# Jackxiini/Tensorflow-distributed-learning

Hardware: AMD Instinct MI355X
Metric: images/sec (whole node) MNIST CNN global_batch=64*N (higher is better)
Workload: dtype fp32; 1 GPU; global_batch=64, parallelism=dp1, engine=fused, communicator=local, variant=reference, process_model=single, communicator_impl=LocalCommunicator, ipc_mode=dmabuf, allreduce=local, steps_per_execution=25, graph_captured=True, input_prefetch_executions=1, allreduce_in_graph=False, replicas_identical=True

## Files before the change

### csrc/kernels/mnist_cnn.hip

```cpp
#include <type_traits>

#include "common.h"
#include "mnist_cnn.h"
#include "optim.h"
#include "xgmi_device.h"

namespace tdl {

struct HeadWeights {
  float wa[10], wb[10], b4[10], b3a, b3b;
};

__device__ __forceinline__ HeadWeights load_head_weights(const MnistArgs& a, int l) {
  HeadWeights hw;
  const float* w4 = a.W + a.ow4;
#pragma unroll
  for (int c = 0; c < 10; ++c) {
    hw.wa[c] = w4[l * 10 + c];
    hw.wb[c] = w4[(l + 64) * 10 + c];
    hw.b4[c] = a.W[a.ob4 + c];
  }
  hw.b3a = a.W[a.ob3 + l];
  hw.b3b = a.W[a.ob3 + l + 64];
  return hw;
// ... 267 lines not shown
    const int mt = T >> 3, nt = T & 7, n = nt * 16 + i;
    if (mt < 100) {
      const int kf = mt * 16 + i;
      const int e4 = a.ow3 + (mt * 16 + 4 * g + (i & 3)) * 128 + nt * 16 + (i & 12);
      const f4 wold = sgd ? ld4(a.W + e4) : zero4();
      const f4 acc = quad_transpose(gemm_tn_buf(b, g, buf_rsrc(a.P2, (unsigned)(b * 1600 * 4)), 1600 * 4, kf * 4,
                                                buf_rsrc(a.dH, (unsigned)(b * 128 * 4)), 128 * 4, n * 4), i & 3);
      if (keep_g) st4(a.G + e4, acc);
      if (xdst != nullptr) st4(xdst + e4, acc);
      if (sgd) st4_sc1(buf_rsrc(a.W, (unsigned)a.nslab * 4u), e4 * 4, wold - lr * acc);
    } else {
      const float wold = sgd ? a.W[a.ob3 + n] : 0.f;
      const auto dhr = buf_rsrc(a.dH, (unsigned)(b * 128 * 4));
      const f4 acc = gemm_tn_buf<true>(b, g, dhr, 0, 0, dhr, 128 * 4, n * 4, i == 0 ? 1.f : 0.f);
      if (g == 0) {
        if (keep_g) a.G[a.ob3 + n] = acc[0];
        if (xdst != nullptr) xdst[a.ob3 + n] = acc[0];
        if (sgd) a.W[a.ob3 + n] = wold - lr * acc[0];
      }
    }
    return;
  }
  const int T3 = T - kD1TasksW3;
  if (T3 < 9) {
    const int c = min(i, 9);
    float wold[4];
#pragma unroll
    for (int r = 0; r < 4; ++r)
      wold[r] = sgd ? a.W[T3 < 8 ? a.ow4 + (T3 * 16 + 4 * g + r) * 10 + c : a.ob4 + c] : 0.f;
    const auto dlr = buf_rsrc(a.dL, (unsigned)(b * kDLStride * 4));
    const int dlc = i < 10 ? i * 4 : 0x40000000;
    const f4 acc = T3 < 8 ? gemm_tn_buf(b, g, buf_rsrc(a.H, (unsigned)(b * 128 * 4)), 128 * 4, (T3 * 16 + i) * 4, dlr,
                                        kDLStride * 4, dlc)
                          : gemm_tn_buf<true>(b, g, dlr, 0, 0, dlr, kDLStride * 4, dlc, i == 0 ? 1.f : 0.f);
    if (i < 10) {
      if (T3 < 8) {
#pragma unroll
        for (int r = 0; r < 4; ++r) {
          const int e = a.ow4 + (T3 * 16 + 4 * g + r) * 10 + i;
          if (keep_g) a.G[e] = acc[r];
          if (xdst != nullptr) xdst[e] = acc[r];
          if (sgd) a.W[e] = wold[r] - lr * acc[r];
        }
      } else if (g == 0) {
        if (keep_g) a.G[a.ob4 + i] = acc[0];
        if (xdst != nullptr) xdst[a.ob4 + i] = acc[0];
        if (sgd) a.W[a.ob4 + i] = wold[0] - lr * acc[0];
      }
    }
  }
}

__device__ __forceinline__ void dp2_task(const MnistArgs& a, int T, int lane) {
  const int i = lane & 15, g = lane >> 4;
  const int b = a.b;
  const int MT = (b + 15) >> 4;
  const int mt = T % MT, nt = T / MT;
  const int row = mt * 16 + i;
  const bool valid = row < b;
  const float* ap = a.dH + (valid ? row : 0) * 128 + 4 * g;
  const float* bp = a.W + a.ow3 + (size_t)(nt * 16 + i) * 128 + 4 * g;
  f4 av[8], bv[8];
#pragma unroll
  for (int s = 0; s < 8; ++s) {
    av[s] = ld4(ap + s * 16);
    bv[s] = ld4(bp + s * 16);
  }
  float p2v[4];
#pragma unroll
  for (int r = 0; r < 4; ++r) p2v[r] = a.P2[(size_t)min(mt * 16 + 4 * g + r, b - 1) * 1600 + nt * 16 + i];
  __builtin_amdgcn_sched_barrier(0);
  const float vm = valid ? 1.f : 0.f;
  f4 acc0 = zero4(), acc1 = zero4();
#pragma unroll
  for (int s = 0; s < 8; ++s) {
    const f4 x = av[s] * vm;
    acc0 = mfma16x16x4(x.x, bv[s].x, acc0);
    acc1 = mfma16x16x4(x.y, bv[s].y, acc1);
    acc0 = mfma16x16x4(x.z, bv[s].z, acc0);
    acc1 = mfma16x16x4(x.w, bv[s].w, acc1);
  }
  const f4 acc = acc0 + acc1;
#pragma unroll
  for (int r = 0; r < 4; ++r) {
    const int rr = mt * 16 + 4 * g + r;
    if (rr < b) a.dP2[(size_t)rr * 1600 + nt * 16 + i] = p2v[r] > 0.f ? acc[r] : 0.f;
  }
}

__global__ __launch_bounds__(256) void k_dense1_bwd(MnistArgs a, int ndp2) {
  const int T = blockIdx.x * 4 + (threadIdx.x >> 6);
  if (T < ndp2) {
    dp2_task(a, T, threadIdx.x & 63);
    return;
  }
  if (T - ndp2 < kDenseTasks) dense_w_task(a, T - ndp2, threadIdx.x & 63, false, 0.f);
}

constexpr int kP1Stride = 36;
constexpr int kDcStride = 80, kDcDim = 15, kP1StrideB = 48;
constexpr int kDgSplit = 80;
__constant__ int kWgradTiles[2][8][2] = {{{0, 6}, {6, 5}, {11, 6}, {0, 0}, {0, 0}, {0, 0}, {0, 0}, {17, 2}},
                                         {{0, 5}, {5, 5}, {10, 5}, {15, 4}, {0, 0}, {0, 0}, {0, 0}, {0, 0}}};
constexpr int kLdsDc = kDcDim * kDcDim * kDcStride;
constexpr int kLdsP1 = 169 * kP1StrideB;
constexpr int kLdsWd = 9 * 16 * 16 * 4;
constexpr int kLdsConvBwd = kLdsDc + kLdsP1 + 784 + kLdsWd + 8 * 10 * 16;

__global__ __launch_bounds__(512) void k_conv_bwd(MnistArgs a) {
  extern __shared__ __attribute__((aligned(16))) float sm[];
  float* dCs = sm;
  float* P1s = dCs + kLdsDc;
  float* Xs = P1s + kLdsP1;
  float* Wd = Xs + 784;
  float* red = Wd + kLdsWd;
  const int tid = threadIdx.x, wave = __builtin_amdgcn_readfirstlane(tid >> 6), lane = tid & 63;
  const int i = lane & 15, g = lane >> 4;
  const int bi = blockIdx.x >> 2, p = blockIdx.x & 3;
  const int h = p & 1, half = p >> 1;
  if (blockIdx.x == 0) {
    for (int r = tid; r < a.b; r += 512) a.cnt[r] = 0u;
    if (tid == 0) a.ep[0] += 1u;
  }
  stamp(a.stamps, 0);
  constexpr int kIdc = (kLdsDc / 4 + 511) / 512, kIp1 = (169 * 8 + 511) / 512, kIwd = (kLdsWd / 4 + 511) / 512;
  f4 vdc[kIdc], vp1[kIp1], vwd[kIwd], vx;
  unsigned qdc[kIdc];
  int sel[kIdc];
  const float* dpb = a.dP2 + (size_t)bi * 1600;
  const unsigned* a2b = reinterpret_cast<const unsigned*>(a.A2 + (size_t)bi * 1600);
#pragma unroll
  for (int j = 0; j < kIdc; ++j) {
    const int e4 = tid + j * 512;
    const int cell = e4 / (kDcStride / 4), c4 = e4 - cell * (kDcStride / 4);
    const int y = cell / kDcDim - 2, x = cell - (cell / kDcDim) * kDcDim - 2;
    const bool in = e4 < kLdsDc / 4 && c4 < 16 && y >= 0 && y < 10 && x >= 0 && x < 10;
    const int o = in ? ((y >> 1) * 5 + (x >> 1)) * 64 + c4 * 4 : 0;
    sel[j] = in ? (y & 1) * 2 + (x & 1) : 4;
    vdc[j] = ld4(dpb + o);
    qdc[j] = a2b[o >> 2];
  }
  const float* p1b = a.P1 + (size_t)bi * 169 * 32;
#pragma unroll
  for (int j = 0; j < kIp1; ++j) {
    const int e4 = min(tid + j * 512, 169 * 8 - 1);
    vp1[j] = ld4(p1b + (e4 >> 3) * 32 + (e4 & 7) * 4);
  }
#pragma unroll
  for (int j = 0; j < kIwd; ++j) {
    const int e4 = min(tid + j * 512, kLdsWd / 4 - 1);
    const int jj = e4 & 15, cq = (e4 >> 4) & 15, tap = e4 >> 8;
    vwd[j] = ld4(a.W + a.ow2 + (size_t)(tap * 32 + 16 * h + jj) * 64 + cq * 4);
  }
  vx = ld4(a.X + (size_t)a.idx[bi] * 784 + min(tid, 195) * 4);
  __builtin_amdgcn_sched_barrier(0);
#pragma unroll
  for (int j = 0; j < kIdc; ++j) {
    const int e4 = tid + j * 512;
    if (e4 < kLdsDc / 4) {
      const unsigned q = qdc[j];
      const unsigned s = (unsigned)sel[j];
      const f4 v = vdc[j];
      st4(dCs + e4 * 4, f4{(q & 0xffu) == s ? v.x : 0.f, ((q >> 8) & 0xffu) == s ? v.y : 0.f,
                           ((q >> 16) & 0xffu) == s ? v.z : 0.f, (q >> 24) == s ? v.w : 0.f});
    }
  }
#pragma unroll
  for (int j = 0; j < kIp1; ++j) {
    const int e4 = tid + j * 512;
    if (e4 < 169 * 8) st4(P1s + (e4 >> 3) * kP1StrideB + (e4 & 7) * 4, vp1[j]);
  }
#pragma unroll
  for (int j = 0; j < kIwd; ++j) {
    const int e4 = tid + j * 512;
    if (e4 < kLdsWd / 4) st4(Wd + e4 * 4, vwd[j]);
  }
  if (tid < 196) st4(Xs + tid * 4, vx);
  stamp(a.stamps, 1);
  __syncthreads();
  stamp(a.stamps, 2);

  {
    const int t0 = kWgradTiles[half][wave][0], ntiles = kWgradTiles[half][wave][1];
    for (int j = 0; j < ntiles; ++j) {
      const int mt = t0 + j;
      const bool bias_tile = mt == 18;
      const int k = mt * 16 + i;
      const int tap = bias_tile ? 0 : k >> 5, ci = k & 31;
      const int kh = tap / 3, kw = tap - kh * 3;
      const float* pa0 = P1s + (kh * 13 + kw + g) * kP1StrideB + ci;
      const float* paS = pa0 + (g >= 2 ? 3 * kP1StrideB : 0);
      const float* pb0 = dCs + (2 * kDcDim + 2 + g) * kDcStride + 16 * p + i;
      const float* pbS = pb0 + (g >= 2 ? 5 * kDcStride : 0);
      const float unit_a = (i == 0) ? 1.f : 0.f;
      auto kloop = [&](auto bias) {
        f4 c0 = zero4(), c1 = zero4();
#pragma unroll
        for (int s0 = 0; s0 < 25; s0 += 5) {
          float av[5], bv[5];
#pragma unroll
          for (int u = 0; u < 5; ++u) {
            const int st = s0 + u, q = (4 * st) / 10, r = (4 * st) % 10;
            const bool strad = r == 8;
            if constexpr (decltype(bias)::value) av[u] = unit_a;
            else av[u] = (strad ? paS : pa0)[(q * 13 + r) * kP1StrideB];
            bv[u] = (strad ? pbS : pb0)[(q * kDcDim + r) * kDcStride];
          }
#pragma unroll
          for (int u = 0; u < 5; ++u) {
            if ((s0 + u) & 1) c1 = mfma16x16x4(av[u], bv[u], c1);
            else c0 = mfma16x16x4(av[u], bv[u], c0);
          }
        }
        return c0 + c1;
      };
      const f4 acc = bias_tile ? kloop(std::true_type{}) : kloop(std::false_type{});
#pragma unroll
      for (int r = 0; r < 4; ++r) {
        const int row = mt * 16 + 4 * g + r;
        if (row < kMnistPart2Rows) a.part2[((size_t)bi * kMnistPart2Rows + row) * 64 + 16 * p + i] = acc[r];
      }
    }
  }

  stamp(a.stamps, 3);
  float dw[10];
#pragma unroll
  for (int j = 0; j < 10; ++j) dw[j] = 0.f;
  const int d = 7 - wave;
  const int pix0 = half ? kDgSplit : 0, pix1 = half ? 169 : kDgSplit;
  if (d < (pix1 - pix0 + 15) / 16) {
    const int P = pix0 + d * 16 + i;
    const bool valid = P < pix1;
    const int Pc = valid ? P : pix0;
    const int ih = Pc / 13, iw = Pc - ih * 13;
    const float* wb = Wd + (g * 16 + i) * 4;
    const int c = 16 * h + i;
    unsigned q1v[4];
#pragma unroll
    for (int r = 0; r < 4; ++r) {
      const int Pr = min(pix0 + d * 16 + 4 * g + r, pix1 - 1);
      q1v[r] = a.A1[((size_t)bi * 169 + Pr) * 32 + c];
    }
    const int ih_lo = (pix0 + d * 16) / 13, ih_hi = min(pix0 + d * 16 + 15, pix1 - 1) / 13;
    const int kh_lo = max(0, ih_lo - 9), kh_hi = min(2, ih_hi);
    f4 acc0 = zero4(), acc1 = zero4();
    for (int kh = kh_lo; kh <= kh_hi; ++kh) {
#pragma unroll
      for (int kw = 0; kw < 3; ++kw) {
        const int tap = kh * 3 + kw;
        const float* ap = dCs + ((ih - kh + 2) * kDcDim + (iw - kw + 2)) * kDcStride + 4 * g;
#pragma unroll
        for (int c0 = 0; c0 < 64; c0 += 16) {
          const f4 av = ld4(ap + c0);
          const f4 bv = ld4(wb + (tap * 16 + c0 / 4) * 64);
          acc0 = mfma16x16x4(av.x, bv.x, acc0);
          acc1 = mfma16x16x4(av.y, bv.y, acc1);
          acc0 = mfma16x16x4(av.z, bv.z, acc0);
          acc1 = mfma16x16x4(av.w, bv.w, acc1);
        }
      }
    }
    const f4 acc = acc0 + acc1;
    stamp(a.stamps, 6);
#pragma unroll
    for (int r = 0; r < 4; ++r) {
      const int Pr = pix0 + d * 16 + 4 * g + r;
      if (Pr < pix1) {
        const float v = P1s[Pr * kP1StrideB + c] > 0.f ? acc[r] : 0.f;
        const unsigned q1 = q1v[r];
        const int ph = Pr / 13, pw = Pr - ph * 13;
        const float* img = Xs + (2 * ph + (q1 >> 1)) * 28 + 2 * pw + (q1 & 1);
#pragma unroll
        for (int kh = 0; kh < 3; ++kh)
#pragma unroll
          for (int kw = 0; kw < 3; ++kw) dw[kh * 3 + kw] = fmaf(img[kh * 28 + kw], v, dw[kh * 3 + kw]);
        dw[9] += v;
      }
    }
  }
#pragma unroll
  for (int j = 0; j < 10; ++j) dw[j] = sum_lane_groups(dw[j]);
  if (g == 0) {
#pragma unroll
    for (int j = 0; j < 10; ++j) red[(wave * 10 + j) * 16 + i] = dw[j];
  }
  stamp(a.stamps, 4);
  __syncthreads();
  stamp(a.stamps, 5);
  if (tid < 160) {
    const int j = tid >> 4, ii = tid & 15;
    float s = 0.f;
#pragma unroll
    for (int w = 2; w < 8; ++w) s += red[(w * 10 + j) * 16 + ii];
    a.part1[((size_t)bi * 2 + half) * kMnistPart1Cols + j * 32 + 16 * h + ii] = s;
  }
}

constexpr int kLdsFwd = 784 + 320 + 169 * kP1Stride + 72 * 16 * 4 + 400 + 169 * 32 / 4 + 400 / 4 + 16 * 128 + 4 + 128 +
                        288 * 16 +
                        kHeadW;
constexpr int kDcF = 15, kDcFStride = 20;
constexpr int kLdsFwdFused = kLdsFwd + kDcF * kDcF * kDcFStride;
__constant__ int kFusedWgradTiles[8][2] = {{0, 2}, {2, 2}, {4, 3}, {7, 3}, {10, 2}, {12, 2}, {14, 2}, {16, 2}};

__device__ __forceinline__ void bwd_stamp(unsigned long long* buf, int k) {
  if (buf != nullptr && (threadIdx.x & 63) == 0)
    buf[(size_t)gridDim.x * 72 + (blockIdx.x * 8 + (threadIdx.x >> 6)) * 4 + k] = __builtin_amdgcn_s_memrealtime();
}

template <int N>
__device__ __forceinline__ void fused_wgrad_tiles(const MnistArgs& a, int bi, int cq, int t0, const float* P1s,
                                                  const float* dCs) {
  const int lane = threadIdx.x & 63, i = lane & 15, g = lane >> 4;
  const float* pa0[N];
#pragma unroll
  for (int u = 0; u < N; ++u) {
    const int k = (t0 + u) * 16 + i;
    const int tap = k >> 5, ci = k & 31;
    const int kh = tap / 3, kw = tap - kh * 3;
    pa0[u] = P1s + (kh * 13 + kw + g) * kP1Stride + ci;
  }
  const int wrapA = g >= 2 ? 3 * kP1Stride : 0, wrapB = g >= 2 ? 5 * kDcFStride : 0;
  const float* pb0 = dCs + (2 * kDcF + 2 + g) * kDcFStride + i;
  f4 acc[N];
#pragma unroll
  for (int u = 0; u < N; ++u) acc[u] = zero4();
  constexpr int kS = 3, kBlocks = (25 + kS - 1) / kS;
  float bv[2][kS], av[2][kS][N];
  auto load = [&](int buf, int blk) {
#pragma unroll
    for (int j = 0; j < kS; ++j) {
      const int st = blk * kS + j;
      if (st >= 25) break;
      const int q = (4 * st) / 10, r = (4 * st) % 10;
      const bool strad = r == 8;
      bv[buf][j] = pb0[(q * kDcF + r) * kDcFStride + (strad ? wrapB : 0)];
#pragma unroll
      for (int u = 0; u < N; ++u) av[buf][j][u] = pa0[u][(q * 13 + r) * kP1Stride + (strad ? wrapA : 0)];
    }
  };
  load(0, 0);
#pragma unroll
  for (int blk = 0; blk < kBlocks; ++blk) {
    if (blk + 1 < kBlocks) load((blk + 1) & 1, blk + 1);
    __builtin_amdgcn_sched_barrier(0);
#pragma unroll
    for (int j = 0; j < kS; ++j) {
      if (blk * kS + j >= 25) break;
#pragma unroll
      for (int u = 0; u < N; ++u) acc[u] = mfma16x16x4(av[blk & 1][j][u], bv[blk & 1][j], acc[u]);
    }
    __builtin_amdgcn_sched_barrier(0);
  }
  const auto rs = buf_rsrc(a.part2 + (size_t)bi * kP2QuadFloats, kP2QuadFloats * 4);
#pragma unroll
  for (int u = 0; u < N; ++u) st4_sc1(rs, ((((t0 + u) * 4 + g) * 64 + 16 * cq + i) * 4) * 4, acc[u]);
}

__device__ __forceinline__ void lds_dgrad_w2(const float* w2d, f4 (&bwd)[9]) {
  const int wave = __builtin_amdgcn_readfirstlane(threadIdx.x >> 6), lane = threadIdx.x & 63;
  const int i = lane & 15, g = lane >> 4, nt = wave >> 2;
#pragma unroll
  for (int tap = 0; tap < 9; ++tap) bwd[tap] = ld4(w2d + (tap * 32 + 16 * nt + i) * 16 + 4 * g);
}

__device__ __forceinline__ void fused_conv_bwd(const MnistArgs& a, int bi, int cq, const float* dp2s,
                                               const uint8_t* a2s, const float* P1s, const uint8_t* a1s,
                                               const float* xs, float* dCs, float* red, const f4 (&bwd)[9]) {
  const int tid = threadIdx.x, wave = __builtin_amdgcn_readfirstlane(tid >> 6), lane = tid & 63;
  const int i = lane & 15, g = lane >> 4;
  bwd_stamp(a.stamps, 0);

  auto wgrad = [&]() {
    const int t0 = kFusedWgradTiles[wave][0], ntiles = kFusedWgradTiles[wave][1];
    if (ntiles == 2) fused_wgrad_tiles<2>(a, bi, cq, t0, P1s, dCs);
    else fused_wgrad_tiles<3>(a, bi, cq, t0, P1s, dCs);
  };
  const bool swap = (a.variant & kMnistVariantStagger) && wave >= 4;
  if (!swap) wgrad();
  bwd_stamp(a.stamps, 1);

  float dw[10];
#pragma unroll
  for (int j = 0; j < 10; ++j) dw[j] = 0.f;
  {
    const int nt = wave >> 2, wt = wave & 3;
    const int ci = 16 * nt + i;
    constexpr int kT = 3;
    f4 acc[kT][2];
    int ih[kT], iw[kT], khlo[kT], khhi[kT];
#pragma unroll
    for (int u = 0; u < kT; ++u) {
      const int t = wt + 4 * u;
      const int Pc = min(t * 16 + i, 168);
      ih[u] = Pc / 13;
      iw[u] = Pc - ih[u] * 13;
      const int ih_lo = min(t * 16, 168) / 13, ih_hi = min(t * 16 + 15, 168) / 13;
      khlo[u] = t < 11 ? max(0, ih_lo - 9) : 3;
      khhi[u] = min(2, ih_hi);
      acc[u][0] = zero4();
      acc[u][1] = zero4();
    }
    float p1v[kT][4];
    unsigned q1v[kT][4];
#pragma unroll
    for (int u = 0; u < kT; ++u)
#pragma unroll
      for (int r = 0; r < 4; ++r) {
        const int Pr = min((wt + 4 * u) * 16 + 4 * g + r, 168);
        p1v[u][r] = P1s[Pr * kP1Stride + ci];
        q1v[u][r] = a1s[Pr * 32 + ci];
      }
    f4 av[2][kT];
    auto load = [&](int buf, int tap) {
      const int kh = tap / 3, kw = tap - kh * 3;
#pragma unroll
      for (int u = 0; u < kT; ++u)
        av[buf][u] = ld4(dCs + ((ih[u] - kh + 2) * kDcF + (iw[u] - kw + 2)) * kDcFStride + 4 * g);
    };
    load(0, 0);
#pragma unroll
    for (int tap = 0; tap < 9; ++tap) {
      if (tap + 1 < 9) load((tap + 1) & 1, tap + 1);
      __builtin_amdgcn_sched_barrier(0);
      const int kh = tap / 3;
      const f4 bv = bwd[tap];
#pragma unroll
      for (int u = 0; u < kT; ++u) {
        if (kh < khlo[u] || kh > khhi[u]) continue;
        const f4 x = av[tap & 1][u];
        acc[u][0] = mfma16x16x4(x.x, bv.x, acc[u][0]);
        acc[u][1] = mfma16x16x4(x.y, bv.y, acc[u][1]);
        acc[u][0] = mfma16x16x4(x.z, bv.z, acc[u][0]);
        acc[u][1] = mfma16x16x4(x.w, bv.w, acc[u][1]);
      }
      __builtin_amdgcn_sched_barrier(0);
    }
#pragma unroll
    for (int u = 0; u < kT; ++u) {
      const int t = wt + 4 * u;
      if (t >= 11) continue;
      const f4 ac = acc[u][0] + acc[u][1];
#pragma unroll
      for (int r = 0; r < 4; ++r) {
        const int Pr = t * 16 + 4 * g + r;
        if (Pr < 169) {
          const float v = p1v[u][r] > 0.f ? ac[r] : 0.f;
          const unsigned q1 = q1v[u][r];
          const int ph = Pr / 13, pw = Pr - ph * 13;
          const float* img = xs + (2 * ph + (q1 >> 1)) * 28 + 2 * pw + (q1 & 1);
#pragma unroll
          for (int kh = 0; kh < 3; ++kh)
#pragma unroll
            for (int kw = 0; kw < 3; ++kw) dw[kh * 3 + kw] = fmaf(img[kh * 28 + kw], v, dw[kh * 3 + kw]);
          dw[9] += v;
        }
      }
    }
  }
  if (swap) wgrad();
  bwd_stamp(a.stamps, 2);
#pragma unroll
  for (int j = 0; j < 10; ++j) dw[j] = sum_lane_groups(dw[j]);
  if (g == 0) {
#pragma unroll
    for (int j = 0; j < 10; ++j) red[(wave * 10 + j) * 16 + i] = dw[j];
  }
  lds_barrier();
  bwd_stamp(a.stamps, 3);
  if (tid < kMnistPart1Cols) {
    const int j = tid >> 5, c = tid & 31, nt = c >> 4, ii = c & 15;
    float sum = 0.f;
#pragma unroll
    for (int w = 0; w < 4; ++w) sum += red[((4 * nt + w) * 10 + j) * 16 + ii];
    a.part1[((size_t)bi * 4 + cq) * kMnistPart1Cols + tid] = sum;
  }
}

__device__ __forceinline__ void store_saved_fwd(const MnistArgs& a, int bi, int cq, const float* P1s,
                                                const uint8_t* a1s, const float* p2s, const uint8_t* a2s,
                                                int t, int nt) {
  for (int e = (a.fused_bwd ? 676 : 0) + t; e < (a.fused_bwd ? 776 : 2 * 338 + 200); e += nt) {
    if (e < 338) {
      const int e4 = cq * 338 + e, pos = e4 >> 3, c4 = (e4 & 7) * 4;
      st4(a.P1 + (size_t)bi * 5408 + e4 * 4, ld4(P1s + pos * kP1Stride + c4));
    } else if (e < 676) {
      const int w = cq * 338 + (e - 338);
      reinterpret_cast<unsigned*>(a.A1 + (size_t)bi * 5408)[w] = reinterpret_cast<const unsigned*>(a1s)[w];
    } else if (e < 776) {
      const int u = e - 676, wo = u >> 2, q = u & 3;
      st4(a.P2 + (size_t)bi * 1600 + wo * 64 + 16 * cq + 4 * q, ld4(p2s + wo * 16 + 4 * q));
    } else {
      const int u = e - 776, wo = u >> 2, q = u & 3;
      *reinterpret_cast<unsigned*>(a.A2 + (size_t)bi * 1600 + wo * 64 + 16 * cq + 4 * q) =
          reinterpret_cast<const unsigned*>(a2s)[wo * 4 + q];
    }
  }
}

__global__ __launch_bounds__(512) void k_fwd_conv(MnistArgs a) {
  extern __shared__ __attribute__((aligned(16))) float sm[];
  float* xs = sm;
  float* w1s = xs + 784;
  float* P1s = w1s + 320;
  float* w2s = P1s + 169 * kP1Stride;
  float* p2s = w2s + 72 * 16 * 4;
  uint8_t* a1s = reinterpret_cast<uint8_t*>(p2s + 400);
  uint8_t* a2s = a1s + 169 * 32;
  float* red = reinterpret_cast<float*>(a2s + 400);
  int* s_last = reinterpret_cast<int*>(red + 16 * 128);
  float* w2d = red + 16 * 128 + 4 + 128;
  float* hws = w2d + 288 * 16;
  float* dCs = hws + kHeadW;
  const int tid = threadIdx.x, wave = tid >> 6, lane = tid & 63;
  const int i = lane & 15, g = lane >> 4;
  int bi = blockIdx.x >> 2, cq = blockIdx.x & 3;
  if ((a.variant & kMnistVariantXcd) && (a.b & 7) == 0) {
    const int x = blockIdx.x & 7, sl = blockIdx.x >> 3;
    bi = x * (a.b >> 3) + (sl >> 2);
    cq = sl & 3;
  }
  if ((a.variant & kMnistVariantPrio) && __builtin_amdgcn_readfirstlane(wave) >= 4) __builtin_amdgcn_s_setprio(1);
  stamp(a.stamps, 0);
  const int sample = a.idx[bi];
  const f4 vx = ld4(a.X + (size_t)sample * 784 + min(tid, 195) * 4);
  const int label = a.Y[sample];
  const float vw1 = tid < 288 ? a.W[a.ow1 + tid] : a.W[a.ob1 + min(tid - 288, 31)];
  f4 vw2[3];
#pragma unroll
  for (int j = 0; j < 3; ++j) {
    const int e = min(tid + j * 512, 1151);
    vw2[j] = ld4(a.W + a.ow2 + (e >> 2) * 64 + 16 * cq + (e & 3) * 4);
  }
  const float b2v = a.W[a.ob2 + 16 * cq + (lane & 15)];
  const uint32_t tag = a.ep[0] + 1u;
  __builtin_amdgcn_sched_barrier(0);
  if (tid < 196) st4(xs + tid * 4, vx);
  if (tid < 320) w1s[tid] = vw1;
#pragma unroll
  for (int j = 0; j < 3; ++j) {
    const int e = tid + j * 512;
    if (e < 1152) {
      const int k = e >> 2, q = e & 3;
      float* d = w2s + ((k >> 2) * 16 + 4 * q) * 4 + (k & 3);
      d[0] = vw2[j].x;
      d[4] = vw2[j].y;
      d[8] = vw2[j].z;
      d[12] = vw2[j].w;
      st4(w2d + k * 16 + 4 * q, vw2[j]);
    }
  }
  stamp(a.stamps, 1);
  __syncthreads();
  stamp(a.stamps, 2);
  const int n4 = (tid & 31) * 4, rg = tid >> 5;
  f4 w3v[25];
  const auto w3r = buf_rsrc(a.W + a.ow3 + (size_t)16 * cq * 128, (unsigned)((1600 - 16 * cq) * 128 * 4));
  const int w3vo = (rg * 128 + n4) * 4;
  auto ldw3 = [&](int j) { w3v[j] = ld4_buf(w3r, w3vo, j * 64 * 128 * 4); };
#pragma unroll
  for (int j = 0; j < 6; ++j) ldw3(j);
  {
    float bw[2][3];
#pragma unroll
    for (int nt = 0; nt < 2; ++nt)
#pragma unroll
      for (int s3 = 0; s3 < 3; ++s3) {
        const int k = 4 * s3 + g;
        bw[nt][s3] = k < 9 ? w1s[k * 32 + nt * 16 + i] : 0.f;
      }
    int tap_off[3];
#pragma unroll
    for (int s3 = 0; s3 < 3; ++s3) {
      const int k = min(4 * s3 + g, 8);
      tap_off[s3] = (k / 3) * 28 + (k % 3);
    }
    const float bias[2] = {w1s[288 + i], w1s[288 + 16 + i]};
    float xa[2][2][3];
    auto load_x = [&](int buf, int it) {
      const int mt0 = wave + 16 * it;
#pragma unroll
      for (int u = 0; u < 2; ++u) {
        const int mt = min(mt0 + 8 * u, 42);
        const int w = mt * 4 + (i >> 2), q = i & 3;
        const int wc = min(w, 168);
        const int y = 2 * (wc / 13) + (q >> 1), x = 2 * (wc % 13) + (q & 1);
        const float* xb = xs + y * 28 + x;
#pragma unroll
        for (int s3 = 0; s3 < 3; ++s3) xa[buf][u][s3] = xb[tap_off[s3]];
      }
    };
    load_x(0, 0);
#pragma unroll
    for (int it = 0; it < 3; ++it) {
      const int mt0 = wave + 16 * it;
      f4 acc[2][2];
#pragma unroll
      for (int u = 0; u < 2; ++u)
#pragma unroll
        for (int nt = 0; nt < 2; ++nt) acc[u][nt] = zero4();
#pragma unroll
      for (int s3 = 0; s3 < 3; ++s3)
#pragma unroll
        for (int u = 0; u < 2; ++u)
#pragma unroll
          for (int nt = 0; nt < 2; ++nt) acc[u][nt] = mfma16x16x4(xa[it & 1][u][s3], bw[nt][s3], acc[u][nt]);
      __builtin_amdgcn_sched_barrier(0);
      if (it < 2) load_x((it + 1) & 1, it + 1);
      __builtin_amdgcn_sched_barrier(0);
      if (it < 2) {
#pragma unroll
        for (int j = 6 + 5 * it; j < 11 + 5 * it; ++j) ldw3(j);
        __builtin_amdgcn_sched_barrier(0);
      }
#pragma unroll
      for (int u = 0; u < 2; ++u) {
        const int wo = (mt0 + 8 * u) * 4 + g;
        if (mt0 + 8 * u >= 43 || wo >= 169) continue;
#pragma unroll
        for (int nt = 0; nt < 2; ++nt) {
          const f4 ac = acc[u][nt];
          float m = ac.x;
          unsigned am = 0;
          if (ac.y > m) { m = ac.y; am = 1; }
          if (ac.z > m) { m = ac.z; am = 2; }
          if (ac.w > m) { m = ac.w; am = 3; }
          const int co = nt * 16 + i;
          const float v = fmaxf(m + bias[nt], 0.f);
          P1s[wo * kP1Stride + co] = v;
          a1s[wo * 32 + co] = (uint8_t)am;
        }
      }
    }
  }
  stamp(a.stamps, 3);
  lds_barrier();
  stamp(a.stamps, 4);
  if (wave < 7) {
    const int wi = wave * 4 + (i >> 2), q = i & 3;
    const bool valid = wi < 25;
    const int wic = valid ? wi : 0;
    const int ph = wic / 5, pw = wic - ph * 5;
    const int oh = 2 * ph + (q >> 1), ow = 2 * pw + (q & 1);
    const float* ab = P1s + (oh * 13 + ow) * kP1Stride + 4 * g;
    const float* bb = w2s + (g * 16 + i) * 4;
    f4 acc0 = zero4(), acc1 = zero4();
#pragma unroll
    for (int kk = 0; kk < 9; ++kk) {
      const int kh = kk / 3, kw = kk % 3;
#pragma unroll
      for (int cb = 0; cb < 32; cb += 16) {
        const f4 av = ld4(ab + (kh * 13 + kw) * kP1Stride + cb);
        const f4 bv = ld4(bb + ((kk * 32 + cb) / 4) * 64);
        acc0 = mfma16x16x4(av.x, bv.x, acc0);
        acc1 = mfma16x16x4(av.y, bv.y, acc1);
        acc0 = mfma16x16x4(av.z, bv.z, acc0);
        acc1 = mfma16x16x4(av.w, bv.w, acc1);
      }
      __builtin_amdgcn_sched_barrier(0);
      ldw3(16 + kk);
      __builtin_amdgcn_sched_barrier(0);
    }
    const f4 acc = acc0 + acc1;
    stamp(a.stamps, 5);
    const int wo = wave * 4 + g;
    if (wo < 25) {
      float m = acc.x;
      unsigned am = 0;
      if (acc.y > m) { m = acc.y; am = 1; }
      if (acc.z > m) { m = acc.z; am = 2; }
      if (acc.w > m) { m = acc.w; am = 3; }
      const float v = fmaxf(m + b2v, 0.f);
      p2s[wo * 16 + i] = v;
      a2s[wo * 16 + i] = (uint8_t)am;
    }
  } else {
#pragma unroll
    for (int j = 16; j < 25; ++j) ldw3(j);
    if (a.head != 0) {
      float hv[23];
#pragma unroll
      for (int u = 0; u < 23; ++u) {
        const int e = min(lane + 64 * u, 1417);
        hv[u] = a.W[e < 1280 ? a.ow4 + e : (e < 1408 ? a.ob3 + (e - 1280) : a.ob4 + (e - 1408))];
      }
#pragma unroll
      for (int u = 0; u < 23; ++u)
        if (lane + 64 * u < 1418) hws[lane + 64 * u] = hv[u];
    }
    if (a.head == 1 && a.dp2_fwd && a.fused_bwd) {
      for (int e4 = lane; e4 < kDcF * kDcF * kDcFStride / 4; e4 += 64) st4(dCs + e4 * 4, zero4());
    }
  }
  __syncthreads();
  {
    f4 hs = zero4();
#pragma unroll
    for (int j = 0; j < 25; ++j) hs += p2s[j * 16 + rg] * w3v[j];
    st4(red + rg * 128 + n4, hs);
  }
  lds_barrier();
  const bool tagged = a.head == 1 && a.dp2_fwd;
  float* sown = red + 16 * 128 + 4;
  if (tid < 32) {
    f4 hsum = zero4();
#pragma unroll
    for (int k = 0; k < 16; ++k) hsum += ld4(red + k * 128 + 4 * tid);
    if (!tagged) {
      st4_sc1(buf_rsrc(a.part3 + ((size_t)cq * a.b + bi) * 128, 512), tid * 16, hsum);
    } else {
      st4(sown + 4 * tid, hsum);
      unsigned long long* p = a.part3t + ((size_t)cq * a.b + bi) * 128 + 4 * tid;
      const unsigned long long tg = (unsigned long long)tag << 32;
      __hip_atomic_store(p, (unsigned long long)__float_as_uint(hsum.x) | tg, __ATOMIC_RELAXED, __HIP_MEMORY_SCOPE_AGENT);
      __hip_atomic_store(p + 1, (unsigned long long)__float_as_uint(hsum.y) | tg, __ATOMIC_RELAXED,
                         __HIP_MEMORY_SCOPE_AGENT);
      __hip_atomic_store(p + 2, (unsigned long long)__float_as_uint(hsum.z) | tg, __ATOMIC_RELAXED,
                         __HIP_MEMORY_SCOPE_AGENT);
      __hip_atomic_store(p + 3, (unsigned long long)__float_as_uint(hsum.w) | tg, __ATOMIC_RELAXED,
                         __HIP_MEMORY_SCOPE_AGENT);
    }
  }
  stamp(a.stamps, 6);
  if (a.head == 0) {
    store_saved_fwd(a, bi, cq, P1s, a1s, p2s, a2s, tid, 512);
    return;
  }
  HeadWeights hw;
  const int uwave = __builtin_amdgcn_readfirstlane(wave);
  if (uwave == 0) hw = lds_head_weights(hws, lane);
  f4 bwd[9];
  if (a.head == 1 && a.dp2_fwd && a.fused_bwd) lds_dgrad_w2(w2d, bwd);

  if (!tagged) {
    asm volatile("s_waitcnt vmcnt(0)" ::: "memory");
    __syncthreads();
    if (tid == 0) {
      const unsigned old = __hip_atomic_fetch_add(a.cnt + bi, 1u, __ATOMIC_RELAXED, __HIP_MEMORY_SCOPE_AGENT);
      s_last[0] = (old & 3u) == 3u;
    }
  }
  lds_barrier();
  const bool last = tagged || s_last[0] != 0;
  float* sdh = red;
  if (last && uwave == 0) {
    if (a.head == 1) head_row(a, bi, lane, label, hw, sdh, tag, tagged ? sown : nullptr, cq, !tagged || cq == kHeadQuarter);
    else head_eval(a, bi, lane, label, hw);
  }
  if (a.head != 1) return;
  if (!last) store_saved_fwd(a, bi, cq, P1s, a1s, p2s, a2s, tid, 512);
  else if (wave != 0) store_saved_fwd(a, bi, cq, P1s, a1s, p2s, a2s, tid - 64, 448);
  if (!a.dp2_fwd) return;
  lds_barrier();
  if (a.fused_bwd) stamp(a.stamps, 7);
  const f4 dh = ld4(sdh + n4);
  float v[25];
  {
    typedef float f2 __attribute__((ext_vector_type(2)));
    const f2 dlo = {dh.x, dh.y}, dhi = {dh.z, dh.w};
#pragma unroll
    for (int j = 0; j < 25; ++j) {
      f2 t = f2{w3v[j].x, w3v[j].y} * dlo;
      t = __builtin_elementwise_fma(f2{w3v[j].z, w3v[j].w}, dhi, t);
      v[j] = t.x + t.y;
    }
  }
  const float d = reduce_scatter32<25>(v, lane);
  const int j = lane & 31;
  if (a.fused_bwd) {
    float val = 0.f;
    if (j < 25) {
      const int kk = j * 16 + rg;
      val = p2s[kk] > 0.f ? d : 0.f;
      const unsigned am = a2s[kk];
      const int ph = (j * 13) >> 6, pw = j - 5 * ph;
      const int y = 2 * ph + (int)(am >> 1), x = 2 * pw + (int)(am & 1u);
      dCs[((y + 2) * kDcF + x + 2) * kDcFStride + rg] = val;
    }
    float sb = rs_swap16(val, val);
    sb += dpp_xor8(sb);
    sb += dpp_mirror8(sb);
    sb += dpp_xor2(sb);
    sb += dpp_xor1(sb);
    if (j == 0) {
      const auto rs = buf_rsrc(a.part2 + (size_t)bi * kP2QuadFloats, kP2QuadFloats * 4);
      st4_sc1(rs, (((kP2Quads - 1) * 64 + 16 * cq + rg) * 4) * 4, f4{sb, 0.f, 0.f, 0.f});
    }
    lds_barrier();
    fused_conv_bwd(a, bi, cq, p2s, a2s, P1s, a1s, xs, dCs, red, bwd);
    return;
  }
  if (j < 25) {
    const int kk = j * 16 + rg;
    a.dP2[(size_t)bi * 1600 + j * 64 + 16 * cq + rg] = p2s[kk] > 0.f ? d : 0.f;
  }
  stamp(a.stamps, 7);
}

__global__ __launch_bounds__(256) void k_finalize(MnistArgs a, int apply_sgd, int ndb, int nbs, int nb2, int nb1) {
  const float lr = *a.lr;
  int blk = blockIdx.x;
  if (blk < ndb) {
    const int T = blk * 4 + (threadIdx.x >> 6);
    if (T < kDenseTasks) dense_w_task(a, T, threadIdx.x & 63, apply_sgd != 0, lr);
    return;
  }
  blk -= ndb;
  if (blk < nbs) {
    const int e = a.ow3 + blk * 256 + threadIdx.x;
    if (e < a.nslab) a.W[e] -= lr * a.G[e];
    return;
  }
  if (blk < nbs + nb2) {
    const int t = (blk - nbs) * 256 + threadIdx.x;
    const int o = t >> 2, sub = t & 3;
    const int n = kMnistPart2Rows * 64;
    float s = 0.f;
    const int oc = min(o, n - 1);
    const int e = (oc >> 6) < 288 ? a.ow2 + oc : a.ob2 + (oc & 63);
    const float wold = apply_sgd ? a.W[e] : 0.f;
    for (int base = 0; base < a.b; base += 64) {
      float v[16];
#pragma unroll
      for (int j = 0; j < 16; ++j) v[j] = a.part2[(size_t)min(base + sub + 4 * j, a.b - 1) * n + oc];
#pragma unroll
      for (int j = 0; j < 16; ++j) s += (base + sub + 4 * j < a.b) ? v[j] : 0.f;
    }
    s += __shfl_xor(s, 1, 64);
    s += __shfl_xor(s, 2, 64);
    if (sub == 0 && o < n) {
      a.G[e] = s;
      if (apply_sgd) a.W[e] = wold - lr * s;
    }
    return;
  }
  const int t = (blk - nbs - nb2) * 256 + threadIdx.x;
  const int o = t >> 4, sub = t & 15;
  const int rows = mnist_part1_rows(a.b, a.fused_bwd != 0);
  float s = 0.f;
  const int oc = min(o, kMnistPart1Cols - 1);
  const int e = oc < 288 ? a.ow1 + oc : a.ob1 + (oc - 288);
  const float wold = apply_sgd ? a.W[e] : 0.f;
  for (int base = 0; base < rows; base += 128) {
    float v[8];
#pragma unroll
    for (int j = 0; j < 8; ++j) v[j] = a.part1[(size_t)min(base + sub + 16 * j, rows - 1) * kMnistPart1Cols + oc];
#pragma unroll
    for (int j = 0; j < 8; ++j) s += (base + sub + 16 * j < rows) ? v[j] : 0.f;
  }
#pragma unroll
  for (int m = 1; m < 16; m <<= 1) s += __shfl_xor(s, m, 64);
  if (sub == 0 && o < kMnistPart1Cols) {
    a.G[e] = s;
    if (apply_sgd) a.W[e] = wold - lr * s;
  }
}

__device__ __forceinline__ void fx_range(const MnistArgs& a, int j, int& lo, int& cnt, int& nseg, int& stride) {
  nseg = 1;
  stride = 0;
  if (j < kFxW3) {
    lo = a.ow3 + (j >> 1) * 2048 + (j & 1) * 64;
    cnt = 64;
    nseg = 16;
    stride = 128;
  } else if (j < kFxW3 + 4) {
    lo = a.ob3 + 32 * (j - kFxW3);
    cnt = 32;
  } else if (j < kFxW3 + 8) {
    lo = a.ow4 + 320 * (j - kFxW3 - 4);
    cnt = 320;
  } else if (j == kFxW3 + 8) {
    lo = a.ob4;
    cnt = 10;
  } else if (j < kFxDense + kFxConv2) {
    const int qd = (j - kFxDense) >> 1, h = (j - kFxDense) & 1;
    if (qd == kP2Quads - 1) {
      lo = a.ob2 + 32 * h;
      cnt = 32;
    } else {
      lo = a.ow2 + qd * 256 + 32 * h;
      cnt = 32;
      nseg = 4;
      stride = 64;
    }
  } else {
    const int q = j - kFxDense - kFxConv2;
    lo = q < 18 ? a.ow1 + q * 16 : a.ob1 + (q - 18) * 16;
    cnt = 16;
  }
}

template <int R>
__device__ __forceinline__ void finalize_x_body(const MnistArgs& a, int apply_sgd, int j);

template <int R, bool LOOP>
__global__ __launch_bounds__(512) void k_finalize_x(MnistArgs a, int apply_sgd) {
  unsigned long long* sb = a.stamps == nullptr ? nullptr
      : a.stamps + (size_t)a.b * 4 * 104 + ((size_t)blockIdx.x * 8 + (threadIdx.x >> 6)) * 2;
  if (sb != nullptr && (threadIdx.x & 63) == 0) sb[0] = __builtin_amdgcn_s_memrealtime();
  if constexpr (LOOP) {
    for (int j = blockIdx.x; j < kFxBlocks; j += gridDim.x) {
      finalize_x_body<R>(a, apply_sgd, j);
      __syncthreads();
    }
  } else {
    finalize_x_body<R>(a, apply_sgd, blockIdx.x);
  }
  if (sb != nullptr && (threadIdx.x & 63) == 0) sb[1] = __builtin_amdgcn_s_memrealtime();
}

template <int R>
__device__ __forceinline__ void finalize_x_body(const MnistArgs& a, int apply_sgd, int j) {
  const int tid = threadIdx.x, wave = tid >> 6, lane = tid & 63;
  const float lr = *a.lr;
  const bool xchg = R > 1 && a.xchg && apply_sgd;
  if (j == 0 && tid == 4 * 64) a.ep[0] += 1u;
  uint32_t e = 0;
  float* xdst = nullptr;
  int64_t half = 0;
  if (xchg) {
    e = __builtin_amdgcn_readfirstlane(a.xa.epoch[j]) + 1u;
    if (xgmi_failed(a.xa.err)) {
      if (tid == 0) a.xa.epoch[j] = e;
      return;
    }
    half = (int64_t)(e & 1u) * 2 * a.xa.cap;
    xdst = a.xa.p.buf[a.xa.rank] + half;
  }
  const bool sgd_local = R == 1 && apply_sgd;
  const bool keep_g = !((sgd_local || xchg) && (a.variant & kMnistVariantNoG));
  if (j < kFxW3) {
    if (wave < 4) dense_w_task(a, (j >> 1) * 8 + (j & 1) * 4 + wave, lane, sgd_local, lr, xdst, keep_g);
  } else if (j < kFxDense) {
// ... 249 lines not shown
```

Before: 2.678 million images/sec.

## Skip dead conv1 row/column 12 and rebalance conv backward tiles per wave

```diff
diff --git a/csrc/kernels/mnist_cnn.hip b/csrc/kernels/mnist_cnn.hip
--- a/csrc/kernels/mnist_cnn.hip
+++ b/csrc/kernels/mnist_cnn.hip
@@ -593,7 +593,9 @@
                         kHeadW;
 constexpr int kDcF = 15, kDcFStride = 20;
 constexpr int kLdsFwdFused = kLdsFwd + kDcF * kDcF * kDcFStride;
-__constant__ int kFusedWgradTiles[8][2] = {{0, 2}, {2, 2}, {4, 3}, {7, 3}, {10, 2}, {12, 2}, {14, 2}, {16, 2}};
+constexpr int kP1Live = 12;
+constexpr int kConv1Tiles = kP1Live * kP1Live / 4;
+__constant__ int kFusedWgradTiles[8][2] = {{0, 2}, {3, 2}, {7, 3}, {12, 3}, {2, 1}, {5, 2}, {10, 2}, {15, 3}};
 
 __device__ __forceinline__ void bwd_stamp(unsigned long long* buf, int k) {
   if (buf != nullptr && (threadIdx.x & 63) == 0)
@@ -666,7 +668,8 @@
   auto wgrad = [&]() {
     const int t0 = kFusedWgradTiles[wave][0], ntiles = kFusedWgradTiles[wave][1];
     if (ntiles == 2) fused_wgrad_tiles<2>(a, bi, cq, t0, P1s, dCs);
-    else fused_wgrad_tiles<3>(a, bi, cq, t0, P1s, dCs);
+    else if (ntiles == 3) fused_wgrad_tiles<3>(a, bi, cq, t0, P1s, dCs);
+    else fused_wgrad_tiles<1>(a, bi, cq, t0, P1s, dCs);
   };
   const bool swap = (a.variant & kMnistVariantStagger) && wave >= 4;
   if (!swap) wgrad();
@@ -675,10 +678,10 @@
   float dw[10];
 #pragma unroll
   for (int j = 0; j < 10; ++j) dw[j] = 0.f;
-  {
-    const int nt = wave >> 2, wt = wave & 3;
+  const int nt = wave >> 2, wt = wave & 3;
+  auto dgrad = [&](auto ktiles) {
+    constexpr int kT = decltype(ktiles)::value;
     const int ci = 16 * nt + i;
-    constexpr int kT = 3;
     f4 acc[kT][2];
     int ih[kT], iw[kT], khlo[kT], khhi[kT];
 #pragma unroll
@@ -749,7 +752,9 @@
         }
       }
     }
-  }
+  };
+  if (wt < 2) dgrad(std::integral_constant<int, 3>{});
+  else dgrad(std::integral_constant<int, 2>{});
   if (swap) wgrad();
   bwd_stamp(a.stamps, 2);
 #pragma unroll
@@ -868,15 +873,19 @@
       tap_off[s3] = (k / 3) * 28 + (k % 3);
     }
     const float bias[2] = {w1s[288 + i], w1s[288 + 16 + i]};
+    const int cwave = __builtin_amdgcn_readfirstlane(wave);
+    static_assert(kConv1Tiles == 4 * 6 + 4 * 3, "slot -> tile map of conv1");
+    auto live = [&](int it, int u) { return cwave < 4 || 2 * it + u < 3; };
+    const int mtb = wave < 4 ? wave : 20 + wave;
     float xa[2][2][3];
     auto load_x = [&](int buf, int it) {
-      const int mt0 = wave + 16 * it;
+      const int mt0 = mtb + 8 * it;
 #pragma unroll
       for (int u = 0; u < 2; ++u) {
-        const int mt = min(mt0 + 8 * u, 42);
-        const int w = mt * 4 + (i >> 2), q = i & 3;
-        const int wc = min(w, 168);
-        const int y = 2 * (wc / 13) + (q >> 1), x = 2 * (wc % 13) + (q & 1);
+        if (!live(it, u)) continue;
+        const int w = (mt0 + 4 * u) * 4 + (i >> 2), q = i & 3;
+        const int ph = w / kP1Live;
+        const int y = 2 * ph + (q >> 1), x = 2 * (w - ph * kP1Live) + (q & 1);
         const float* xb = xs + y * 28 + x;
 #pragma unroll
         for (int s3 = 0; s3 < 3; ++s3) xa[buf][u][s3] = xb[tap_off[s3]];
@@ -885,7 +894,7 @@
     load_x(0, 0);
 #pragma unroll
     for (int it = 0; it < 3; ++it) {
-      const int mt0 = wave + 16 * it;
+      const int mt0 = mtb + 8 * it;
       f4 acc[2][2];
 #pragma unroll
       for (int u = 0; u < 2; ++u)
@@ -894,9 +903,11 @@
 #pragma unroll
       for (int s3 = 0; s3 < 3; ++s3)
 #pragma unroll
-        for (int u = 0; u < 2; ++u)
+        for (int u = 0; u < 2; ++u) {
+          if (!live(it, u)) continue;
 #pragma unroll
           for (int nt = 0; nt < 2; ++nt) acc[u][nt] = mfma16x16x4(xa[it & 1][u][s3], bw[nt][s3], acc[u][nt]);
+        }
       __builtin_amdgcn_sched_barrier(0);
       if (it < 2) load_x((it + 1) & 1, it + 1);
       __builtin_amdgcn_sched_barrier(0);
@@ -907,8 +918,10 @@
       }
 #pragma unroll
       for (int u = 0; u < 2; ++u) {
-        const int wo = (mt0 + 8 * u) * 4 + g;
-        if (mt0 + 8 * u >= 43 || wo >= 169) continue;
+        if (!live(it, u)) continue;
+        const int w = (mt0 + 4 * u) * 4 + g;
+        const int ph = w / kP1Live;
+        const int wo = ph * 13 + (w - ph * kP1Live);
 #pragma unroll
         for (int nt = 0; nt < 2; ++nt) {
           const f4 ac = acc[u][nt];
@@ -922,6 +935,15 @@
           P1s[wo * kP1Stride + co] = v;
           a1s[wo * 32 + co] = (uint8_t)am;
         }
+      }
+    }
+    if (cwave >= 4) {
+      const int e = tid - 256;
+      if (e < 25 * 8) {
+        const int c = e >> 3, c4 = e & 7;
+        const int cell = c < 13 ? 12 * 13 + c : (c - 13) * 13 + 12;
+        st4(P1s + cell * kP1Stride + 4 * c4, zero4());
+        reinterpret_cast<unsigned*>(a1s)[cell * 8 + c4] = 0u;
       }
     }
   }
```

New measurement: 2.748 million images/sec (median of 6 runs). 2.6% higher.
